# A-Nasiri-M/sap3d_tensorflow

Hardware: AMD Instinct MI355X
Metric: clips/s (16x112x112 fwd+bwd) (higher is better)
Workload: dtype f32

## Files before the change

### sap3d_tensorflow_amd/csrc/elementwise.hip

```cpp
#include "p3d_kernels.h"
#include "det_reduce.h"
#define P3D_SEED(a) ((a).seed_dev ? *(a).seed_dev : (a).seed)

namespace {

__device__ __forceinline__ float4 ld4(const float* p) { return *reinterpret_cast<const float4*>(p); }
__device__ __forceinline__ void st4(float* p, float4 v) { *reinterpret_cast<float4*>(p) = v; }
__device__ __forceinline__ float4 f4(float a) { return make_float4(a, a, a, a); }
__device__ __forceinline__ float4 fma4(float4 a, float4 b, float4 c) {
    return make_float4(fmaf(a.x, b.x, c.x), fmaf(a.y, b.y, c.y), fmaf(a.z, b.z, c.z), fmaf(a.w, b.w, c.w));
}
__device__ __forceinline__ float4 add4(float4 a, float4 b) { return make_float4(a.x + b.x, a.y + b.y, a.z + b.z, a.w + b.w); }
__device__ __forceinline__ float4 sub4(float4 a, float4 b) { return make_float4(a.x - b.x, a.y - b.y, a.z - b.z, a.w - b.w); }
__device__ __forceinline__ float4 mul4(float4 a, float4 b) { return make_float4(a.x * b.x, a.y * b.y, a.z * b.z, a.w * b.w); }
__device__ __forceinline__ float relu1(float v) { return v > 0.f ? v : (v != v ? v : 0.f); }
__device__ __forceinline__ float4 relu4(float4 a) { return make_float4(relu1(a.x), relu1(a.y), relu1(a.z), relu1(a.w)); }
__device__ __forceinline__ float4 gate4(float4 g, float4 pre) {
    return make_float4(pre.x > 0.f ? g.x : 0.f, pre.y > 0.f ? g.y : 0.f, pre.z > 0.f ? g.z : 0.f, pre.w > 0.f ? g.w : 0.f);
}

__device__ __forceinline__ float u01(unsigned long long seed, unsigned long long idx) {
    unsigned long long z = seed + 0x9E3779B97F4A7C15ull * (idx + 1);
    z = (z ^ (z >> 30)) * 0xBF58476D1CE4E5B9ull;
    z = (z ^ (z >> 27)) * 0x94D049BB133111EBull;
    z ^= z >> 31;
    return (float)(z >> 40) * (1.0f / 16777216.0f);
}
__device__ __forceinline__ float4 dropmask4(unsigned long long seed, long long e0, float rate, float scale) {
    return make_float4(u01(seed, e0) >= rate ? scale : 0.f, u01(seed, e0 + 1) >= rate ? scale : 0.f,
                       u01(seed, e0 + 2) >= rate ? scale : 0.f, u01(seed, e0 + 3) >= rate ? scale : 0.f);
}

static_assert(P3D_STAT_REPLICAS == 16, "finalize kernels fold 16 replicas with 4 shuffle steps");
__device__ __forceinline__ double fold16(double v) {
#pragma unroll
    for (int o = 8; o > 0; o >>= 1) v += __shfl_xor(v, o);
    return v;
}
template <int LPC>
__global__ __launch_bounds__(256) void bn_finalize_kernel(BnParams bn, double invM, int use_batch, int update_moving, float eps) {
    P3D_CHAIN_PRIO();
    const int r = threadIdx.x % LPC;
    const int c = blockIdx.x * (256 / LPC) + threadIdx.x / LPC;
    const bool ok = c < bn.C;
    double s1 = 0.0, s2 = 0.0;
    if (use_batch) {
        if (ok) {
            const float2* part = reinterpret_cast<const float2*>(bn.statpart) + c;
#pragma unroll 4
            for (int q = r; q < bn.nparts; q += LPC) {
                const float2 v = part[(size_t)q * bn.C];
                s1 += (double)v.x; s2 += (double)v.y;
            }
        }
#pragma unroll
        for (int o = LPC / 2; o > 0; o >>= 1) { s1 += __shfl_xor(s1, o); s2 += __shfl_xor(s2, o); }
    }
    if (!ok || r) return;
    double mean, var;
    if (use_batch) {
        mean = s1 * invM;
        var = s2 * invM - mean * mean;
        if (var < 0.0) var = 0.0;
        if (update_moving) {
            bn.moving_mean[c] -= (bn.moving_mean[c] - (float)mean) * (1.0f - 0.99f);
            bn.moving_var[c] -= (bn.moving_var[c] - (float)var) * (1.0f - 0.99f);
        }
    } else {
        mean = bn.moving_mean[c];
        var = bn.moving_var[c];
    }
    const double inv = 1.0 / sqrt(var + (double)eps);
    const float sc = (float)((double)bn.gamma[c] * inv);
    bn.scale[c] = sc;
    bn.shift[c] = (float)((double)bn.beta[c] - mean * (double)bn.gamma[c] * inv);
    bn.mean[c] = (float)mean;
    bn.invstd[c] = (float)inv;
}

__global__ __launch_bounds__(256) void bn_stats_kernel(const float* y, int ld, long long M, int C, float* statpart) {
    P3D_CHAIN_PRIO();
    __shared__ float red[256][8];
    const int c4n = C >> 2;
    const int rpi = 256 / c4n;
    const int tid = threadIdx.x;
    const int sub = tid / c4n;
    const int cg = tid - sub * c4n;
    const int c = cg << 2;
    float4 s1 = f4(0.f), s2 = f4(0.f);
    if (sub < rpi)
        for (long long row = (long long)blockIdx.x * rpi + sub; row < M; row += (long long)gridDim.x * rpi) {
            const float4 v = ld4(y + row * ld + c);
            s1 = add4(s1, v);
            s2 = fma4(v, v, s2);
        }
    float* r = red[tid];
    r[0] = s1.x; r[1] = s1.y; r[2] = s1.z; r[3] = s1.w; r[4] = s2.x; r[5] = s2.y; r[6] = s2.z; r[7] = s2.w;
    __syncthreads();
    if (tid < c4n) {
        float t[8];
#pragma unroll
        for (int q = 0; q < 8; ++q) t[q] = 0.f;
        for (int s = 0; s < rpi; ++s)
#pragma unroll
            for (int q = 0; q < 8; ++q) t[q] += red[s * c4n + tid][q];
        float* st = statpart + (size_t)blockIdx.x * 2 * C;
#pragma unroll
        for (int q = 0; q < 4; ++q) { st[2 * (c + q) + 0] = t[q]; st[2 * (c + q) + 1] = t[4 + q]; }
    }
}

template <int MODE>
__global__ __launch_bounds__(256) void bn_apply_kernel(BnApplyArgs a) {
    p3d_warm_kernarg_lines<(int)(sizeof(BnApplyArgs) / 64)>();
    P3D_CHAIN_PRIO();
    const int c4n = a.C >> 2;
    const long long total = a.M * c4n;
    for (long long i = (long long)blockIdx.x * blockDim.x + threadIdx.x; i < total; i += (long long)gridDim.x * blockDim.x) {
        const long long row = i / c4n;
        const int c = (int)(i - row * c4n) << 2;
        float4 v = fma4(ld4(a.scale1 + c), ld4(a.y1 + row * a.ld1 + c), ld4(a.shift1 + c));
        float4 z;
        if (MODE == 0) z = relu4(v);
        else if (MODE == 1) z = relu4(add4(v, ld4(a.y2 + row * a.ld2 + c)));
        else if (MODE == 2) z = relu4(add4(v, fma4(ld4(a.scale2 + c), ld4(a.y2 + row * a.ld2 + c), ld4(a.shift2 + c))));
        else if (MODE == 3) z = add4(relu4(v), relu4(fma4(ld4(a.scale2 + c), ld4(a.y2 + row * a.ld2 + c), ld4(a.shift2 + c))));
        else z = add4(ld4(a.y2 + row * a.ld2 + c), relu4(v));
        if (a.drop_scale > 0.f) z = mul4(z, dropmask4(P3D_SEED(a), row * a.C + c, a.drop_rate, a.drop_scale));
        st4(a.z + row * a.ldz + c, z);
    }
}

__device__ __forceinline__ void bn_fold64(const BnParams& bn, int c0, double invM, int use_batch, int update_moving, float eps, bool publish,
                                          float* sc_lds, float* sh_lds) {
    const int ch = c0 + (threadIdx.x >> 2), r = threadIdx.x & 3;
    double s1 = 0.0, s2 = 0.0;
    if (use_batch) {
        const float2* part = reinterpret_cast<const float2*>(bn.statpart) + ch;
#pragma unroll 8
        for (int q = r; q < bn.nparts; q += 4) {
            const float2 v = part[(size_t)q * bn.C];
            s1 += (double)v.x; s2 += (double)v.y;
        }
        s1 += __shfl_xor(s1, 1); s2 += __shfl_xor(s2, 1);
        s1 += __shfl_xor(s1, 2); s2 += __shfl_xor(s2, 2);
    }
    if (r) return;
    double mean, var;
    if (use_batch) {
        mean = s1 * invM;
        var = s2 * invM - mean * mean;
        if (var < 0.0) var = 0.0;
        if (publish && update_moving) {
            bn.moving_mean[ch] -= (bn.moving_mean[ch] - (float)mean) * (1.0f - 0.99f);
            bn.moving_var[ch] -= (bn.moving_var[ch] - (float)var) * (1.0f - 0.99f);
        }
    } else {
        mean = bn.moving_mean[ch];
        var = bn.moving_var[ch];
    }
    const double inv = 1.0 / sqrt(var + (double)eps);
    const float sc = (float)((double)bn.gamma[ch] * inv);
    const float sh = (float)((double)bn.beta[ch] - mean * (double)bn.gamma[ch] * inv);
    sc_lds[ch - c0] = sc; sh_lds[ch - c0] = sh;
    if (publish) { bn.scale[ch] = sc; bn.shift[ch] = sh; bn.mean[ch] = (float)mean; bn.invstd[ch] = (float)inv; }
}

template <int MODE>
__global__ __launch_bounds__(256) void bn_fold_apply_kernel(BnApplyArgs a, BnParams bn1, BnParams bn2, double invM, int batch1, int batch2,
                                                           int update_moving, float eps, int rows_per_block) {
    p3d_warm_kernarg_lines<(int)((sizeof(BnApplyArgs) + 2 * sizeof(BnParams)) / 64)>();
    P3D_CHAIN_PRIO();
    constexpr bool TWO = (MODE == 2 || MODE == 3);
    __shared__ __attribute__((aligned(16))) float sc1[64], sh1[64], sc2[64], sh2[64];
    const int c0 = blockIdx.y * 64;
    const bool publish = blockIdx.x == 0;
    bn_fold64(bn1, c0, invM, batch1, update_moving, eps, publish, sc1, sh1);
    if (TWO) bn_fold64(bn2, c0, invM, batch2, update_moving, eps, publish, sc2, sh2);
    __syncthreads();
    const int cl = (threadIdx.x & 15) << 2, c = c0 + cl;
    const float4 s1v = ld4(sc1 + cl), h1v = ld4(sh1 + cl);
    float4 s2v = f4(0.f), h2v = f4(0.f);
    if (TWO) { s2v = ld4(sc2 + cl); h2v = ld4(sh2 + cl); }
    const long long r0 = (long long)blockIdx.x * rows_per_block;
    const long long r1 = r0 + rows_per_block < a.M ? r0 + rows_per_block : a.M;
    for (long long row = r0 + (threadIdx.x >> 4); row < r1; row += 16) {
        const float4 v = fma4(s1v, ld4(a.y1 + row * a.ld1 + c), h1v);
        float4 z;
        if (MODE == 0) z = relu4(v);
        else if (MODE == 1) z = relu4(add4(v, ld4(a.y2 + row * a.ld2 + c)));
        else if (MODE == 2) z = relu4(add4(v, fma4(s2v, ld4(a.y2 + row * a.ld2 + c), h2v)));
        else if (MODE == 3) z = add4(relu4(v), relu4(fma4(s2v, ld4(a.y2 + row * a.ld2 + c), h2v)));
        else z = add4(ld4(a.y2 + row * a.ld2 + c), relu4(v));
        st4(a.z + row * a.ldz + c, z);
    }
}

template <int MODE>
__device__ __forceinline__ void bn_bwd_gates(const BnBwdArgs& a, long long row, int c, float4& g1, float4& g2,
                                             float4& y1, float4& y2) {
    float4 dz = ld4(a.dz + row * a.lddz + c);
    if (a.drop_scale > 0.f) dz = mul4(dz, dropmask4(P3D_SEED(a), row * a.C + c, a.drop_rate, a.drop_scale));
    y1 = ld4(a.y1 + row * a.ld1 + c);
    const float4 v1 = fma4(ld4(a.scale1 + c), y1, ld4(a.shift1 + c));
    y2 = f4(0.f);
    if (MODE == 0) { g1 = gate4(dz, v1); g2 = f4(0.f); }
    else if (MODE == 1) { y2 = ld4(a.y2 + row * a.ld2 + c); g1 = gate4(dz, add4(v1, y2)); g2 = g1; }
    else if (MODE == 2) {
        y2 = ld4(a.y2 + row * a.ld2 + c);
        const float4 v2 = fma4(ld4(a.scale2 + c), y2, ld4(a.shift2 + c));
        g1 = gate4(dz, add4(v1, v2)); g2 = g1;
    } else if (MODE == 3) {
        y2 = ld4(a.y2 + row * a.ld2 + c);
        const float4 v2 = fma4(ld4(a.scale2 + c), y2, ld4(a.shift2 + c));
        g1 = gate4(dz, v1); g2 = gate4(dz, v2);
    } else { g1 = gate4(dz, v1); g2 = dz; }
}

template <int MODE>
__global__ __launch_bounds__(256) void bn_bwd_reduce_kernel(BnBwdArgs a) {
    p3d_warm_kernarg_lines<(int)(sizeof(BnBwdArgs) / 64)>();
    P3D_CHAIN_PRIO();
    constexpr bool TWO = (MODE == 2 || MODE == 3);
    __shared__ float red[256][TWO ? 16 : 8];
    const int c4n = a.C >> 2;
    const int rpi = 256 / c4n;
    const int tid = threadIdx.x;
    const int sub = tid / c4n;
    const int cg = tid - sub * c4n;
    const int c = cg << 2;
    const bool active = sub < rpi;
    float4 s1 = f4(0.f), sx1 = f4(0.f), s2 = f4(0.f), sx2 = f4(0.f);
    if (active) {
        const float4 m1 = ld4(a.mean1 + c), i1 = ld4(a.invstd1 + c);
        float4 m2 = f4(0.f), i2 = f4(0.f);
        if (TWO) { m2 = ld4(a.mean2 + c); i2 = ld4(a.invstd2 + c); }
        const long long stride = (long long)gridDim.x * rpi;
        float4 t1 = f4(0.f), tx1 = f4(0.f), t2 = f4(0.f), tx2 = f4(0.f);
        long long row = (long long)blockIdx.x * rpi + sub;
        for (; row + stride < a.M; row += 2 * stride) {
            float4 g1, g2, y1, y2, h1, h2, z1, z2;
            bn_bwd_gates<MODE>(a, row, c, g1, g2, y1, y2);
            bn_bwd_gates<MODE>(a, row + stride, c, h1, h2, z1, z2);
            s1 = add4(s1, g1);
            sx1 = fma4(g1, mul4(sub4(y1, m1), i1), sx1);
            t1 = add4(t1, h1);
            tx1 = fma4(h1, mul4(sub4(z1, m1), i1), tx1);
            if (TWO) {
                s2 = add4(s2, g2);
                sx2 = fma4(g2, mul4(sub4(y2, m2), i2), sx2);
                t2 = add4(t2, h2);
                tx2 = fma4(h2, mul4(sub4(z2, m2), i2), tx2);
            }
        }
        if (row < a.M) {
            float4 g1, g2, y1, y2;
            bn_bwd_gates<MODE>(a, row, c, g1, g2, y1, y2);
            s1 = add4(s1, g1);
            sx1 = fma4(g1, mul4(sub4(y1, m1), i1), sx1);
            if (TWO) {
                s2 = add4(s2, g2);
                sx2 = fma4(g2, mul4(sub4(y2, m2), i2), sx2);
            }
        }
        s1 = add4(s1, t1); sx1 = add4(sx1, tx1);
        if (TWO) { s2 = add4(s2, t2); sx2 = add4(sx2, tx2); }
    }
    float* r = red[tid];
    r[0] = s1.x; r[1] = s1.y; r[2] = s1.z; r[3] = s1.w; r[4] = sx1.x; r[5] = sx1.y; r[6] = sx1.z; r[7] = sx1.w;
    if (TWO) { r[8] = s2.x; r[9] = s2.y; r[10] = s2.z; r[11] = s2.w; r[12] = sx2.x; r[13] = sx2.y; r[14] = sx2.z; r[15] = sx2.w; }
    __syncthreads();
    if (tid < c4n) {
        constexpr int NV = TWO ? 16 : 8;
        float t[NV];
#pragma unroll
        for (int q = 0; q < NV; ++q) t[q] = 0.f;
        for (int s = 0; s < rpi; ++s)
#pragma unroll
            for (int q = 0; q < NV; ++q) t[q] += red[s * c4n + tid][q];
        float* p1 = a.part1 + ((size_t)blockIdx.x * a.C + c) * 2;
#pragma unroll
        for (int q = 0; q < 4; ++q) { p1[2 * q] = t[q]; p1[2 * q + 1] = t[4 + q]; }
        if (TWO) {
            float* p2 = a.part2 + ((size_t)blockIdx.x * a.C + c) * 2;
#pragma unroll
            for (int q = 0; q < 4; ++q) { p2[2 * q] = t[8 + q]; p2[2 * q + 1] = t[12 + q]; }
        }
    }
}

template <int LPC>
__global__ __launch_bounds__(256) void bn_bwd_finalize_kernel(BnBwdArgs a, int two) {
    p3d_warm_kernarg_lines<(int)(sizeof(BnBwdArgs) / 64)>();
    P3D_CHAIN_PRIO();
    const int r = threadIdx.x % LPC;
    const int c = blockIdx.x * (256 / LPC) + threadIdx.x / LPC;
    const bool ok = c < a.C;
    const double invM = 1.0 / (double)a.M;
    double s1 = 0.0, s2 = 0.0, t1 = 0.0, t2 = 0.0;
    if (ok) {
        const float2* p1 = reinterpret_cast<const float2*>(a.part1) + c;
        const float2* p2 = reinterpret_cast<const float2*>(a.part2) + c;
#pragma unroll 4
        for (int q = r; q < a.nparts; q += LPC) {
            const float2 v = p1[(size_t)q * a.C];
            s1 += (double)v.x; s2 += (double)v.y;
            if (two) { const float2 w = p2[(size_t)q * a.C]; t1 += (double)w.x; t2 += (double)w.y; }
        }
    }
#pragma unroll
    for (int o = LPC / 2; o > 0; o >>= 1) {
        s1 += __shfl_xor(s1, o); s2 += __shfl_xor(s2, o);
        if (two) { t1 += __shfl_xor(t1, o); t2 += __shfl_xor(t2, o); }
    }
    if (!ok || r) return;
    a.dbeta1[c] = (float)s1; a.dgamma1[c] = (float)s2;
    a.coef1[2 * c] = (float)(s1 * invM); a.coef1[2 * c + 1] = (float)(s2 * invM);
    if (two) {
        a.dbeta2[c] = (float)t1; a.dgamma2[c] = (float)t2;
        a.coef2[2 * c] = (float)(t1 * invM); a.coef2[2 * c + 1] = (float)(t2 * invM);
    }
}

__global__ __launch_bounds__(256) void bn_grad_finalize_kernel(BnGradFold f) {
    P3D_CHAIN_PRIO();
    const int r = threadIdx.x & 15;
    const int c = blockIdx.x * 16 + (threadIdx.x >> 4);
    const bool ok = c < f.C;
    double sg = 0.0, sgx = 0.0;
    if (ok) {
        const float2* part = reinterpret_cast<const float2*>(f.part) + c;
#pragma unroll 4
        for (int q = r; q < f.nparts; q += 16) {
            const float2 v = part[(size_t)q * f.C];
            sg += (double)v.x; sgx += (double)v.y;
        }
    }
    sg = fold16(sg); sgx = fold16(sgx);
    if (!ok || r) return;
    const float inv = f.invstd[c];
    const float c1 = (float)(sg * f.inv_m), c2 = (float)(sgx * f.inv_m);
    const float k1 = f.gamma[c] * inv;
    const float k2 = -k1 * inv * c2;
    const float k3 = -k1 * c1 - k2 * f.mean[c];
    f.coef[c] = k1; f.coef[f.C + c] = k2; f.coef[2 * f.C + c] = k3;
    f.dgamma[c] = (float)sgx; f.dbeta[c] = (float)sg;
}

__device__ __forceinline__ void ldcoef(const float* coef, int c, float4& c1, float4& c2) {
    const float4 lo = ld4(coef + 2 * c), hi = ld4(coef + 2 * c + 4);
    c1 = make_float4(lo.x, lo.z, hi.x, hi.z);
    c2 = make_float4(lo.y, lo.w, hi.y, hi.w);
}

template <int MODE>
__global__ __launch_bounds__(256) void bn_bwd_apply_kernel(BnBwdArgs a) {
    p3d_warm_kernarg_lines<(int)(sizeof(BnBwdArgs) / 64)>();
    P3D_CHAIN_PRIO();
    constexpr bool TWO = (MODE == 2 || MODE == 3);
    const int c4n = a.C >> 2;
    const long long total = a.M * c4n;
    const long long gtid = (long long)blockIdx.x * blockDim.x + threadIdx.x;
    for (long long i = gtid; i < total; i += (long long)gridDim.x * blockDim.x) {
        const long long row = i / c4n;
        const int c = (int)(i - row * c4n) << 2;
        float4 g1, g2, y1, y2;
        bn_bwd_gates<MODE>(a, row, c, g1, g2, y1, y2);
        {
            const float4 k = mul4(ld4(a.gamma1 + c), ld4(a.invstd1 + c));
            float4 d;
            if (a.batch1) {
                const float4 xh = mul4(sub4(y1, ld4(a.mean1 + c)), ld4(a.invstd1 + c));
                float4 c1, c2;
                ldcoef(a.coef1, c, c1, c2);
                d = mul4(k, sub4(sub4(g1, c1), mul4(xh, c2)));
            } else d = mul4(k, g1);
            float* dst = a.dy1 + row * a.lddy1 + c;
            if (a.acc1) d = add4(d, ld4(dst));
            st4(dst, d);
        }
        if (MODE != 0) {
            float4 d;
            if (TWO) {
                const float4 k = mul4(ld4(a.gamma2 + c), ld4(a.invstd2 + c));
                if (a.batch2) {
                    const float4 xh = mul4(sub4(y2, ld4(a.mean2 + c)), ld4(a.invstd2 + c));
                    float4 c1, c2;
                    ldcoef(a.coef2, c, c1, c2);
                    d = mul4(k, sub4(sub4(g2, c1), mul4(xh, c2)));
                } else d = mul4(k, g2);
            } else d = g2;
            float* dst = a.dy2 + row * a.lddy2 + c;
            if (a.acc2) d = add4(d, ld4(dst));
            st4(dst, d);
        }
    }
}

__global__ __launch_bounds__(256) void maxpool_fwd_kernel(PoolArgs a) {
    p3d_warm_kernarg_lines<(int)(sizeof(PoolArgs) / 64)>();
    P3D_CHAIN_PRIO();
    const int c4n = a.C >> 2;
    const long long total = (long long)a.N * a.Do * a.Ho * a.Wo * c4n;
    for (long long i = (long long)blockIdx.x * blockDim.x + threadIdx.x; i < total; i += (long long)gridDim.x * blockDim.x) {
        long long pos = i / c4n;
        const int c = (int)(i - pos * c4n) << 2;
        const long long opos = pos;
        const int ow = (int)(pos % a.Wo); pos /= a.Wo;
        const int oh = (int)(pos % a.Ho); pos /= a.Ho;
        const int od = (int)(pos % a.Do); const int n = (int)(pos / a.Do);
        float4 best = f4(-INFINITY);
        unsigned bx = 0, by = 0, bz = 0, bw = 0;
        bool none = true;
        for (int kd = 0; kd < a.kd; ++kd) {
            const int id = od * a.sd - a.pd + kd;
            if ((unsigned)id >= (unsigned)a.Di) continue;
            for (int kh = 0; kh < a.kh; ++kh) {
                const int ih = oh * a.sh - a.ph + kh;
                if ((unsigned)ih >= (unsigned)a.Hi) continue;
                for (int kw = 0; kw < a.kw; ++kw) {
                    const int iw = ow * a.sw - a.pw + kw;
                    if ((unsigned)iw >= (unsigned)a.Wi) continue;
                    const float4 v = ld4(a.x + ((((long long)n * a.Di + id) * a.Hi + ih) * a.Wi + iw) * a.ldx + c);
                    const unsigned t = (unsigned)((kd * a.kh + kh) * a.kw + kw);
                    if (none || v.x > best.x || (v.x != v.x && best.x == best.x)) { best.x = v.x; bx = t; }
                    if (none || v.y > best.y || (v.y != v.y && best.y == best.y)) { best.y = v.y; by = t; }
                    if (none || v.z > best.z || (v.z != v.z && best.z == best.z)) { best.z = v.z; bz = t; }
                    if (none || v.w > best.w || (v.w != v.w && best.w == best.w)) { best.w = v.w; bw = t; }
                    none = false;
                }
            }
        }
        st4(a.y + opos * a.ldy + c, best);
        if (a.idx) a.idx[opos * c4n + (c >> 2)] = bx | (by << 8) | (bz << 16) | (bw << 24);
    }
}

template <int KIND>
__device__ __forceinline__ float loss_term(float z, float p, float t, int through_sigmoid, float& g) {
    if (KIND == 1) {
        g = (through_sigmoid ? p : 1.f / (1.f + expf(-z))) - t;
        return fmaxf(z, 0.f) - z * t + log1pf(expf(-fabsf(z)));
    }
    const float d = p - t;
    const float ad = fabsf(d);
    const bool quad = KIND == 0 && ad < 1.f;
    g = quad ? d : (d > 0.f ? 1.f : (d < 0.f ? -1.f : (d != d ? d : 0.f)));
    if (through_sigmoid) g *= p * (1.f - p);
    return KIND == 2 ? ad : (quad ? 0.5f * d * d : ad - 0.5f);
}

template <int KIND>
__device__ __forceinline__ void loss_body(const float* logits, const float* pred, const float* target, long long n,
                                          double* loss_out, float* dl, int through_sigmoid, int vec4, double* part,
                                          unsigned* counter) {
    __shared__ double wsum[4];
    __shared__ int last_flag;
    double acc = 0.0;
    const bool need_z = KIND == 1, need_p = KIND != 1 || through_sigmoid;
    const long long gtid = (long long)blockIdx.x * blockDim.x + threadIdx.x, gsz = (long long)gridDim.x * blockDim.x;
// ... 269 lines not shown
        for (long long e = a + threadIdx.x; e < a4; e += 256) one(e);
        for (long long e = b4 + threadIdx.x; e < b; e += 256) one(e);
        acc = p3d_block_sum<true>(acc, wsum);
        if (threadIdx.x == 0) p3d_store_wt(part, (size_t)k, acc);
    }
    if (nfold <= 0) return;
    if (!p3d_last_block_wt(counter, gridDim.x, &last_flag)) return;
    double s = 0.0;
    for (int k = threadIdx.x; k < nfold; k += 256) s += part[k];
    const double sumsq = p3d_block_sum<true>(s, wsum);
    if (threadIdx.x == 0) {
        const double norm = sqrt(sumsq), cn = (double)clip;
        float scale;
        if (!(norm - norm == 0.0)) scale = __builtin_nanf("");
        else if (cn - cn != 0.0) scale = 1.f;
        else scale = (float)(cn / fmax(norm, cn));
        res[0] = sumsq; res[1] = norm;
        *reinterpret_cast<float*>(res + 2) = scale;
    }
}

__global__ __launch_bounds__(256) void add_inplace_kernel(float* dst, int lddst, const float* src, int ldsrc, long long M, int C, int copy) {
    const int c4n = C >> 2;
    const long long total = M * c4n;
    for (long long i = (long long)blockIdx.x * blockDim.x + threadIdx.x; i < total; i += (long long)gridDim.x * blockDim.x) {
        const long long row = i / c4n;
        const int c = (int)(i - row * c4n) << 2;
        float4 v = ld4(src + row * ldsrc + c);
        if (!copy) v = add4(v, ld4(dst + row * lddst + c));
        st4(dst + row * lddst + c, v);
    }
}

__global__ __launch_bounds__(256) void fill_uniform_kernel(float* p, long long n, float lo, float hi, unsigned long long seed) {
    for (long long i = (long long)blockIdx.x * blockDim.x + threadIdx.x; i < n; i += (long long)gridDim.x * blockDim.x)
        p[i] = lo + (hi - lo) * u01(seed, (unsigned long long)i);
}

__global__ __launch_bounds__(256) void fill_trunc_normal_kernel(float* p, long long n, float stddev, unsigned long long seed) {
    for (long long i = (long long)blockIdx.x * blockDim.x + threadIdx.x; i < n; i += (long long)gridDim.x * blockDim.x) {
        float z = 0.f;
        for (int k = 0; k < 32; ++k) {
            const unsigned long long e = 2ull * (unsigned long long)(i + (long long)k * n);
            const float u1 = fmaxf(u01(seed, e), 1e-12f), u2 = u01(seed, e + 1);
            z = sqrtf(-2.f * logf(u1)) * cosf(6.2831853071795865f * u2);
            if (fabsf(z) <= 2.f) break;
            z = 0.f;
        }
        p[i] = stddev * z;
    }
}

__global__ __launch_bounds__(256) void colsum_kernel(const float* dy, int ld, long long M, int C, float* out, float* part,
                                                     unsigned* counters) {
    __shared__ int last_flag;
    const int c = blockIdx.y * blockDim.x + threadIdx.x;
    float acc = 0.f;
    if (c < C) {
        long long row = blockIdx.x;
        const long long st = gridDim.x;
        for (; row + 7 * st < M; row += 8 * st) {
            float v[8];
#pragma unroll
            for (int u = 0; u < 8; ++u) v[u] = dy[(row + u * st) * ld + c];
#pragma unroll
            for (int u = 0; u < 8; ++u) acc += v[u];
        }
        for (; row < M; row += st) acc += dy[row * ld + c];
        p3d_store_wt(part, (size_t)blockIdx.x * C + c, acc);
    }
    if (!p3d_last_block_wt(counters + blockIdx.y, gridDim.x, &last_flag)) return;
    if (c >= C) return;
    float t = 0.f;
    unsigned b = 0;
    for (; b + 7 < gridDim.x; b += 8) {
        float v[8];
#pragma unroll
        for (int u = 0; u < 8; ++u) v[u] = part[(size_t)(b + u) * C + c];
#pragma unroll
        for (int u = 0; u < 8; ++u) t += v[u];
    }
    for (; b < gridDim.x; ++b) t += part[(size_t)b * C + c];
    out[c] += t;
}

__global__ __launch_bounds__(256) void colsum4_kernel(const float* __restrict__ dy, int ld, long long M, int C, float* out,
                                                      float* part, unsigned* counters) {
    __shared__ float4 red[256];
    __shared__ int last_flag;
    const int L = C >> 2, R = 256 / L;
    const int lane = threadIdx.x % L, rs = threadIdx.x / L;
    const bool live = rs < R;
    float4 acc = make_float4(0.f, 0.f, 0.f, 0.f);
    if (live) {
        const long long stride = (long long)gridDim.x * R;
        long long row = (long long)blockIdx.x * R + rs;
        const float* base = dy + lane * 4;
        for (; row + 7 * stride < M; row += 8 * stride) {
            float4 v[8];
#pragma unroll
            for (int u = 0; u < 8; ++u) v[u] = *reinterpret_cast<const float4*>(base + (row + u * stride) * ld);
#pragma unroll
            for (int u = 0; u < 8; ++u) { acc.x += v[u].x; acc.y += v[u].y; acc.z += v[u].z; acc.w += v[u].w; }
        }
        for (; row < M; row += stride) {
            const float4 v = *reinterpret_cast<const float4*>(base + row * ld);
            acc.x += v.x; acc.y += v.y; acc.z += v.z; acc.w += v.w;
        }
    }
    red[threadIdx.x] = acc;
    __syncthreads();
    if (threadIdx.x < L) {
        float4 t = red[threadIdx.x];
        for (int r = 1; r < R; ++r) { const float4 v = red[r * L + threadIdx.x]; t.x += v.x; t.y += v.y; t.z += v.z; t.w += v.w; }
        p3d_store_wt4(part, (size_t)blockIdx.x * C + threadIdx.x * 4, t);
    }
    if (!p3d_last_block_wt(counters, gridDim.x, &last_flag)) return;
    acc = make_float4(0.f, 0.f, 0.f, 0.f);
    if (live) {
        const float* src = part + lane * 4;
        unsigned b = rs;
        for (; b + 7u * R < gridDim.x; b += 8u * R) {
            float4 v[8];
#pragma unroll
            for (int u = 0; u < 8; ++u) v[u] = *reinterpret_cast<const float4*>(src + (size_t)(b + u * R) * C);
#pragma unroll
            for (int u = 0; u < 8; ++u) { acc.x += v[u].x; acc.y += v[u].y; acc.z += v[u].z; acc.w += v[u].w; }
        }
        for (; b < gridDim.x; b += R) {
            const float4 v = *reinterpret_cast<const float4*>(src + (size_t)b * C);
            acc.x += v.x; acc.y += v.y; acc.z += v.z; acc.w += v.w;
        }
    }
    __syncthreads();
    red[threadIdx.x] = acc;
    __syncthreads();
    if (threadIdx.x < L) {
        float4 t = red[threadIdx.x];
        for (int r = 1; r < R; ++r) { const float4 v = red[r * L + threadIdx.x]; t.x += v.x; t.y += v.y; t.z += v.z; t.w += v.w; }
        float4* o = reinterpret_cast<float4*>(out + threadIdx.x * 4);
        float4 cur = *o;
        cur.x += t.x; cur.y += t.y; cur.z += t.z; cur.w += t.w;
        *o = cur;
    }
}

inline unsigned grid_for(long long total, int per_block = 256, int cap = 4096) {
    long long b = (total + per_block - 1) / per_block;
    if (b < 1) b = 1;
    if (b > cap) b = cap;
    return (unsigned)b;
}

}

hipError_t p3d_bn_finalize(const BnParams& bn, long M, int use_batch, int update_moving, float eps, hipStream_t s) {
    if (use_batch && (!bn.statpart || bn.nparts < 1)) return hipErrorInvalidValue;
    if (use_batch && bn.nparts > 64)
        hipLaunchKernelGGL(bn_finalize_kernel<64>, dim3((bn.C + 3) / 4), dim3(256), 0, s, bn, 1.0 / (double)M, use_batch, update_moving, eps);
    else
        hipLaunchKernelGGL(bn_finalize_kernel<16>, dim3((bn.C + 15) / 16), dim3(256), 0, s, bn, 1.0 / (double)M, use_batch, update_moving, eps);
    return hipGetLastError();
}

int p3d_bn_stats_parts(long M, int C) {
    if ((C & 3) || C > 1024 || C < 4) return 0;
    const int rpi = 256 / (C >> 2);
    long long blocks = (M + (long long)rpi * 8 - 1) / ((long long)rpi * 8);
    if (blocks < 1) blocks = 1;
    if (blocks > 512) blocks = 512;
    return (int)blocks;
}

hipError_t p3d_bn_stats(const float* y, int ld, long M, int C, float* statpart, hipStream_t s) {
    if ((C & 3) || C > 1024 || (ld & 3)) return hipErrorInvalidValue;
    const long long blocks = p3d_bn_stats_parts(M, C);
    hipLaunchKernelGGL(bn_stats_kernel, dim3((unsigned)blocks), dim3(256), 0, s, y, ld, (long long)M, C, statpart);
    return hipGetLastError();
}

hipError_t p3d_bn_apply(const BnApplyArgs& a, hipStream_t s) {
    if ((a.C & 3) || (a.ld1 & 3) || (a.ldz & 3)) return hipErrorInvalidValue;
    const unsigned g = grid_for(a.M * (a.C >> 2));
    switch (a.mode) {
        case 0: hipLaunchKernelGGL(bn_apply_kernel<0>, dim3(g), dim3(256), 0, s, a); break;
        case 1: hipLaunchKernelGGL(bn_apply_kernel<1>, dim3(g), dim3(256), 0, s, a); break;
        case 2: hipLaunchKernelGGL(bn_apply_kernel<2>, dim3(g), dim3(256), 0, s, a); break;
        case 3: hipLaunchKernelGGL(bn_apply_kernel<3>, dim3(g), dim3(256), 0, s, a); break;
        case 4: hipLaunchKernelGGL(bn_apply_kernel<4>, dim3(g), dim3(256), 0, s, a); break;
        default: return hipErrorInvalidValue;
    }
    return hipGetLastError();
}

bool p3d_bn_fold_apply_ok(long M, int C, int nparts1, int nparts2, float drop_scale) {
    static const bool off = p3d_tune_env("P3D_BN_FOLD_APPLY") && atoi(p3d_tune_env("P3D_BN_FOLD_APPLY")) == 0;
    return !off && (C % 64) == 0 && nparts1 <= 128 && nparts2 <= 128 && M >= 1024 && !(drop_scale > 0.f);
}
hipError_t p3d_bn_fold_apply(const BnApplyArgs& a, const BnParams& bn1, const BnParams& bn2, int batch1, int batch2, int update_moving,
                             float eps, hipStream_t s) {
    const bool two = a.mode == 2 || a.mode == 3;
    if ((a.ld1 & 3) || (a.ldz & 3) || !p3d_bn_fold_apply_ok(a.M, a.C, batch1 ? bn1.nparts : 0, two && batch2 ? bn2.nparts : 0, a.drop_scale))
        return hipErrorInvalidValue;
    if ((batch1 && (!bn1.statpart || bn1.nparts < 1)) || (two && batch2 && (!bn2.statpart || bn2.nparts < 1))) return hipErrorInvalidValue;
    const int groups = a.C / 64;
    int chunks = 256 / groups;
    if (chunks < 1) chunks = 1;
    long rows = (a.M + chunks - 1) / chunks;
    rows = (rows + 15) / 16 * 16;
    chunks = (int)((a.M + rows - 1) / rows);
    const dim3 g((unsigned)chunks, (unsigned)groups);
    const double invM = 1.0 / (double)a.M;
#define P3D_FA(M_) case M_: hipLaunchKernelGGL(bn_fold_apply_kernel<M_>, g, dim3(256), 0, s, a, bn1, bn2, invM, batch1, batch2, update_moving, eps, (int)rows); break;
    switch (a.mode) { P3D_FA(0) P3D_FA(1) P3D_FA(2) P3D_FA(3) P3D_FA(4) default: return hipErrorInvalidValue; }
#undef P3D_FA
    return hipGetLastError();
}

int p3d_bn_bwd_parts(long M, int C) {
    if ((C & 3) || C > 1024 || C < 4) return 0;
    const int rpi = 256 / (C >> 2);
    long long blocks = (M + (long long)rpi * 8 - 1) / ((long long)rpi * 8);
    if (blocks < 1) blocks = 1;
    if (blocks > 512) blocks = 512;
    return (int)blocks;
}

hipError_t p3d_bn_bwd_reduce(const BnBwdArgs& a, hipStream_t s) {
    if ((a.C & 3) || a.C > 1024 || !a.part1 || a.nparts != p3d_bn_bwd_parts(a.M, a.C)) return hipErrorInvalidValue;
    const unsigned g = (unsigned)a.nparts;
    switch (a.mode) {
        case 0: hipLaunchKernelGGL(bn_bwd_reduce_kernel<0>, dim3(g), dim3(256), 0, s, a); break;
        case 1: hipLaunchKernelGGL(bn_bwd_reduce_kernel<1>, dim3(g), dim3(256), 0, s, a); break;
        case 2: hipLaunchKernelGGL(bn_bwd_reduce_kernel<2>, dim3(g), dim3(256), 0, s, a); break;
        case 3: hipLaunchKernelGGL(bn_bwd_reduce_kernel<3>, dim3(g), dim3(256), 0, s, a); break;
        case 4: hipLaunchKernelGGL(bn_bwd_reduce_kernel<4>, dim3(g), dim3(256), 0, s, a); break;
        default: return hipErrorInvalidValue;
    }
    return hipGetLastError();
}

hipError_t p3d_bn_bwd_finalize(const BnBwdArgs& a, hipStream_t s) {
    const int two = (a.mode == 2 || a.mode == 3) ? 1 : 0;
    if (a.nparts >= 64) hipLaunchKernelGGL(bn_bwd_finalize_kernel<64>, dim3((a.C + 3) / 4), dim3(256), 0, s, a, two);
    else hipLaunchKernelGGL(bn_bwd_finalize_kernel<16>, dim3((a.C + 15) / 16), dim3(256), 0, s, a, two);
    return hipGetLastError();
}

hipError_t p3d_bn_grad_finalize(const BnGradFold& f, hipStream_t s) {
    if (!f.part || f.nparts <= 0) return hipErrorInvalidValue;
    hipLaunchKernelGGL(bn_grad_finalize_kernel, dim3((f.C + 15) / 16), dim3(256), 0, s, f);
    return hipGetLastError();
}

hipError_t p3d_bn_bwd_apply(const BnBwdArgs& a, hipStream_t s) {
    if (a.C & 3) return hipErrorInvalidValue;
    unsigned g = grid_for(a.M * (a.C >> 2));
    switch (a.mode) {
        case 0: hipLaunchKernelGGL(bn_bwd_apply_kernel<0>, dim3(g), dim3(256), 0, s, a); break;
        case 1: hipLaunchKernelGGL(bn_bwd_apply_kernel<1>, dim3(g), dim3(256), 0, s, a); break;
        case 2: hipLaunchKernelGGL(bn_bwd_apply_kernel<2>, dim3(g), dim3(256), 0, s, a); break;
        case 3: hipLaunchKernelGGL(bn_bwd_apply_kernel<3>, dim3(g), dim3(256), 0, s, a); break;
        case 4: hipLaunchKernelGGL(bn_bwd_apply_kernel<4>, dim3(g), dim3(256), 0, s, a); break;
        default: return hipErrorInvalidValue;
    }
    return hipGetLastError();
}

hipError_t p3d_maxpool_fwd(const PoolArgs& a, hipStream_t s) {
    if (a.C & 3) return hipErrorInvalidValue;
    const long long total = (long long)a.N * a.Do * a.Ho * a.Wo * (a.C >> 2);
    hipLaunchKernelGGL(maxpool_fwd_kernel, dim3(grid_for(total)), dim3(256), 0, s, a);
    return hipGetLastError();
}

__device__ __forceinline__ bool pool_hit(float v, float y) { return v == y || (v != v && y != y); }
__global__ __launch_bounds__(256) void maxpool_bwd_disjoint_kernel(PoolArgs a, int accumulate) {
    p3d_warm_kernarg_lines<(int)(sizeof(PoolArgs) / 64)>();
    P3D_CHAIN_PRIO();
    const int c4n = a.C >> 2;
    const long long total = (long long)a.N * a.Do * a.Ho * a.Wo * c4n;
    for (long long i = (long long)blockIdx.x * blockDim.x + threadIdx.x; i < total; i += (long long)gridDim.x * blockDim.x) {
        long long pos = i / c4n;
        const int c = (int)(i - pos * c4n) << 2;
        const long long opos = pos;
        const int ow = (int)(pos % a.Wo); pos /= a.Wo;
        const int oh = (int)(pos % a.Ho); pos /= a.Ho;
        const int od = (int)(pos % a.Do); const int n = (int)(pos / a.Do);
        const float4 g = ld4(a.dy + opos * a.lddy + c);
        const float4 y = ld4(a.y + opos * a.ldy + c);
        float4 left = g;
        bool done[4] = {false, false, false, false};
        for (int kd = 0; kd < a.kd; ++kd)
            for (int kh = 0; kh < a.kh; ++kh)
                for (int kw = 0; kw < a.kw; ++kw) {
                    const long long ipos = (((long long)n * a.Di + od * a.sd + kd) * a.Hi + oh * a.sh + kh) * a.Wi + ow * a.sw + kw;
                    const float4 v = ld4(a.x + ipos * a.ldx + c);
                    float4 d = f4(0.f);
                    if (!done[0] && pool_hit(v.x, y.x)) { d.x = left.x; done[0] = true; }
                    if (!done[1] && pool_hit(v.y, y.y)) { d.y = left.y; done[1] = true; }
                    if (!done[2] && pool_hit(v.z, y.z)) { d.z = left.z; done[2] = true; }
                    if (!done[3] && pool_hit(v.w, y.w)) { d.w = left.w; done[3] = true; }
                    float* dst = a.dx + ipos * a.lddx + c;
                    if (accumulate) d = add4(d, ld4(dst));
                    st4(dst, d);
                }
    }
}

__global__ __launch_bounds__(256) void maxpool_bwd_gather_kernel(PoolArgs a, int accumulate) {
    p3d_warm_kernarg_lines<(int)(sizeof(PoolArgs) / 64)>();
    P3D_CHAIN_PRIO();
    const int c4n = a.C >> 2;
    const long long total = (long long)a.N * a.Di * a.Hi * a.Wi * c4n;
    for (long long i = (long long)blockIdx.x * blockDim.x + threadIdx.x; i < total; i += (long long)gridDim.x * blockDim.x) {
        long long pos = i / c4n;
        const int c = (int)(i - pos * c4n) << 2;
        const long long ipos = pos;
        const int iw = (int)(pos % a.Wi); pos /= a.Wi;
        const int ih = (int)(pos % a.Hi); pos /= a.Hi;
        const int id = (int)(pos % a.Di); const int n = (int)(pos / a.Di);
        const int pdv = id + a.pd, phv = ih + a.ph, pwv = iw + a.pw;
        float4 acc = f4(0.f);
        if (a.kd <= 2 * a.sd && a.kh <= 2 * a.sh && a.kw <= 2 * a.sw) {
            int od2[2], oh2[2], ow2[2];
            bool vd[2], vh[2], vw[2];
#pragma unroll
            for (int q = 0; q < 2; ++q) {
                od2[q] = pdv / a.sd - q; vd[q] = od2[q] >= 0 && od2[q] < a.Do && pdv - od2[q] * a.sd < a.kd;
                oh2[q] = phv / a.sh - q; vh[q] = oh2[q] >= 0 && oh2[q] < a.Ho && phv - oh2[q] * a.sh < a.kh;
                ow2[q] = pwv / a.sw - q; vw[q] = ow2[q] >= 0 && ow2[q] < a.Wo && pwv - ow2[q] * a.sw < a.kw;
            }
            unsigned wd[8]; float4 g8[8]; unsigned t8[8]; bool ok[8];
#pragma unroll
            for (int q = 0; q < 8; ++q) {
                const int qd = q >> 2, qh = (q >> 1) & 1, qw = q & 1;
                ok[q] = vd[qd] && vh[qh] && vw[qw];
                t8[q] = (unsigned)(((pdv - od2[qd] * a.sd) * a.kh + (phv - oh2[qh] * a.sh)) * a.kw + (pwv - ow2[qw] * a.sw));
                const long long opos = ok[q] ? (((long long)n * a.Do + od2[qd]) * a.Ho + oh2[qh]) * a.Wo + ow2[qw] : 0;
                wd[q] = ok[q] ? a.idx[opos * c4n + (c >> 2)] : 0xffffffffu;
                g8[q] = ok[q] ? ld4(a.dy + opos * a.lddy + c) : f4(0.f);
            }
#pragma unroll
            for (int q = 0; q < 8; ++q) {
                if (!ok[q]) continue;
                const unsigned w = wd[q], t = t8[q];
                if ((w & 255u) == t) acc.x += g8[q].x;
                if (((w >> 8) & 255u) == t) acc.y += g8[q].y;
                if (((w >> 16) & 255u) == t) acc.z += g8[q].z;
                if ((w >> 24) == t) acc.w += g8[q].w;
            }
        } else
        for (int od = pdv / a.sd; od >= 0 && pdv - od * a.sd < a.kd; --od) {
            if (od >= a.Do) continue;
            for (int oh = phv / a.sh; oh >= 0 && phv - oh * a.sh < a.kh; --oh) {
                if (oh >= a.Ho) continue;
                for (int ow = pwv / a.sw; ow >= 0 && pwv - ow * a.sw < a.kw; --ow) {
                    if (ow >= a.Wo) continue;
                    const unsigned t = (unsigned)(((pdv - od * a.sd) * a.kh + (phv - oh * a.sh)) * a.kw + (pwv - ow * a.sw));
                    const long long opos = (((long long)n * a.Do + od) * a.Ho + oh) * a.Wo + ow;
                    const unsigned w = a.idx[opos * c4n + (c >> 2)];
                    const float4 g = ld4(a.dy + opos * a.lddy + c);
                    if ((w & 255u) == t) acc.x += g.x;
                    if (((w >> 8) & 255u) == t) acc.y += g.y;
                    if (((w >> 16) & 255u) == t) acc.z += g.z;
                    if ((w >> 24) == t) acc.w += g.w;
                }
            }
        }
        float* dst = a.dx + ipos * a.lddx + c;
        if (accumulate) acc = add4(acc, ld4(dst));
        st4(dst, acc);
    }
}

bool p3d_maxpool_disjoint(const PoolArgs& a) {
    return a.kd == a.sd && a.kh == a.sh && a.kw == a.sw && a.pd == 0 && a.ph == 0 && a.pw == 0 &&
           a.Do * a.sd == a.Di && a.Ho * a.sh == a.Hi && a.Wo * a.sw == a.Wi;
}

hipError_t p3d_maxpool_bwd_disjoint(const PoolArgs& a, int accumulate, hipStream_t s) {
    if ((a.C & 3) || !p3d_maxpool_disjoint(a)) return hipErrorInvalidValue;
    const long long total = (long long)a.N * a.Do * a.Ho * a.Wo * (a.C >> 2);
    hipLaunchKernelGGL(maxpool_bwd_disjoint_kernel, dim3(grid_for(total)), dim3(256), 0, s, a, accumulate);
    return hipGetLastError();
}


static uintptr_t low4(const void* q) { return reinterpret_cast<uintptr_t>(q) & 15; }

LaunchDesc p3d_loss_desc(const LossArgs& a) {
    const double n = (double)a.n;
    const bool ts = a.through_sigmoid != 0;
    if (a.kind == 1) return {"sigmoid_ce_kernel", n * (ts ? 8.0 : 11.0), n * (ts ? 16.0 : 12.0)};
    if (a.kind == 2) return {"l1_loss_kernel", n * (ts ? 6.0 : 3.0), n * 12.0};
    return {"smooth_l1_kernel", 0, 12.0 * n};
}

// ... 239 lines not shown
```

Before: 538.0.

## Batch BN partial-stat loads and prefetch activations ahead of stat fold

Adds specialized paths across the BN kernels that issue all partial-sum loads up front in fixed-size unrolled batches instead of a strided loop, so the finalize kernels avoid serialized memory latency. The fold-apply kernel prefetches its first activation rows before the stat fold and sync, overlapping those loads with the reduction. The backward reduce gains a short-chain path that loads up to eight rows per thread into registers before accumulating. This costs more registers and clamped redundant loads, and the new paths can be disabled by environment variables in tuning builds.

```diff
diff --git a/sap3d_tensorflow_amd/csrc/elementwise.hip b/sap3d_tensorflow_amd/csrc/elementwise.hip
--- a/sap3d_tensorflow_amd/csrc/elementwise.hip
+++ b/sap3d_tensorflow_amd/csrc/elementwise.hip
@@ -37,20 +37,51 @@
     for (int o = 8; o > 0; o >>= 1) v += __shfl_xor(v, o);
     return v;
 }
-template <int LPC>
+template <int NB, int LPC, bool TWO>
+__device__ __forceinline__ void bn_lane_batch(const float2* p1, const float2* p2, int r, int nparts, int C, double& s1, double& s2,
+                                              double& t1, double& t2) {
+    float2 v[NB], w[NB];
+#pragma unroll
+    for (int k = 0; k < NB; ++k) {
+        const int q = r + k * LPC;
+        const size_t at = (size_t)(q < nparts ? q : nparts - 1) * C;
+        v[k] = p1[at];
+        if (TWO) w[k] = p2[at];
+    }
+#pragma unroll
+    for (int k = 0; k < NB; ++k)
+        if (r + k * LPC < nparts) {
+            s1 += (double)v[k].x; s2 += (double)v[k].y;
+            if (TWO) { t1 += (double)w[k].x; t2 += (double)w[k].y; }
+        }
+}
+template <int NB0, int LPC, bool TWO>
+__device__ __forceinline__ void bn_lane_tiers(const float2* p1, const float2* p2, int r, int nparts, int C, double& s1, double& s2,
+                                              double& t1, double& t2) {
+    if (nparts <= NB0 * LPC) bn_lane_batch<NB0, LPC, TWO>(p1, p2, r, nparts, C, s1, s2, t1, t2);
+    else if (nparts <= 2 * NB0 * LPC) bn_lane_batch<2 * NB0, LPC, TWO>(p1, p2, r, nparts, C, s1, s2, t1, t2);
+    else bn_lane_batch<4 * NB0, LPC, TWO>(p1, p2, r, nparts, C, s1, s2, t1, t2);
+}
+template <int LPC, bool BATCH>
 __global__ __launch_bounds__(256) void bn_finalize_kernel(BnParams bn, double invM, int use_batch, int update_moving, float eps) {
     P3D_CHAIN_PRIO();
     const int r = threadIdx.x % LPC;
     const int c = blockIdx.x * (256 / LPC) + threadIdx.x / LPC;
     const bool ok = c < bn.C;
+    constexpr int NB0 = LPC == 64 ? 2 : 1;
     double s1 = 0.0, s2 = 0.0;
     if (use_batch) {
         if (ok) {
             const float2* part = reinterpret_cast<const float2*>(bn.statpart) + c;
+            if (BATCH && bn.nparts <= 4 * NB0 * LPC) {
+                double t1 = 0.0, t2 = 0.0;
+                bn_lane_tiers<NB0, LPC, false>(part, part, r, bn.nparts, bn.C, s1, s2, t1, t2);
+            } else {
 #pragma unroll 4
-            for (int q = r; q < bn.nparts; q += LPC) {
-                const float2 v = part[(size_t)q * bn.C];
-                s1 += (double)v.x; s2 += (double)v.y;
+                for (int q = r; q < bn.nparts; q += LPC) {
+                    const float2 v = part[(size_t)q * bn.C];
+                    s1 += (double)v.x; s2 += (double)v.y;
+                }
             }
         }
 #pragma unroll
@@ -132,15 +163,20 @@
 }
 
 __device__ __forceinline__ void bn_fold64(const BnParams& bn, int c0, double invM, int use_batch, int update_moving, float eps, bool publish,
-                                          float* sc_lds, float* sh_lds) {
+                                          float* sc_lds, float* sh_lds, bool batch) {
     const int ch = c0 + (threadIdx.x >> 2), r = threadIdx.x & 3;
     double s1 = 0.0, s2 = 0.0;
     if (use_batch) {
         const float2* part = reinterpret_cast<const float2*>(bn.statpart) + ch;
+        if (batch && bn.nparts <= 128) {
+            double t1 = 0.0, t2 = 0.0;
+            bn_lane_tiers<8, 4, false>(part, part, r, bn.nparts, bn.C, s1, s2, t1, t2);
+        } else {
 #pragma unroll 8
-        for (int q = r; q < bn.nparts; q += 4) {
-            const float2 v = part[(size_t)q * bn.C];
-            s1 += (double)v.x; s2 += (double)v.y;
+            for (int q = r; q < bn.nparts; q += 4) {
+                const float2 v = part[(size_t)q * bn.C];
+                s1 += (double)v.x; s2 += (double)v.y;
+            }
         }
         s1 += __shfl_xor(s1, 1); s2 += __shfl_xor(s2, 1);
         s1 += __shfl_xor(s1, 2); s2 += __shfl_xor(s2, 2);
@@ -167,32 +203,60 @@
 }
 
 template <int MODE>
+__device__ __forceinline__ float4 bn_apply_z(float4 y1, float4 y2, float4 s1v, float4 h1v, float4 s2v, float4 h2v) {
+    const float4 v = fma4(s1v, y1, h1v);
+    if (MODE == 0) return relu4(v);
+    else if (MODE == 1) return relu4(add4(v, y2));
+    else if (MODE == 2) return relu4(add4(v, fma4(s2v, y2, h2v)));
+    else if (MODE == 3) return add4(relu4(v), relu4(fma4(s2v, y2, h2v)));
+    else return add4(y2, relu4(v));
+}
+
+template <int MODE, bool EARLY>
 __global__ __launch_bounds__(256) void bn_fold_apply_kernel(BnApplyArgs a, BnParams bn1, BnParams bn2, double invM, int batch1, int batch2,
                                                            int update_moving, float eps, int rows_per_block) {
     p3d_warm_kernarg_lines<(int)((sizeof(BnApplyArgs) + 2 * sizeof(BnParams)) / 64)>();
     P3D_CHAIN_PRIO();
     constexpr bool TWO = (MODE == 2 || MODE == 3);
+    constexpr int PRE = 4;
     __shared__ __attribute__((aligned(16))) float sc1[64], sh1[64], sc2[64], sh2[64];
     const int c0 = blockIdx.y * 64;
     const bool publish = blockIdx.x == 0;
-    bn_fold64(bn1, c0, invM, batch1, update_moving, eps, publish, sc1, sh1);
-    if (TWO) bn_fold64(bn2, c0, invM, batch2, update_moving, eps, publish, sc2, sh2);
+    const int cl = (threadIdx.x & 15) << 2, c = c0 + cl;
+    const long long r0 = (long long)blockIdx.x * rows_per_block;
+    const long long r1 = r0 + rows_per_block < a.M ? r0 + rows_per_block : a.M;
+    long long row = r0 + (threadIdx.x >> 4);
+    float4 py1[PRE], py2[PRE];
+    auto load_trips = [&]() {
+#pragma unroll
+        for (int k = 0; k < PRE; ++k) {
+            const long long rk = row + 16 * k < r1 ? row + 16 * k : r1 - 1;
+            py1[k] = ld4(a.y1 + rk * a.ld1 + c);
+            py2[k] = MODE != 0 ? ld4(a.y2 + rk * a.ld2 + c) : f4(0.f);
+        }
+    };
+    if (EARLY) load_trips();
+    bn_fold64(bn1, c0, invM, batch1, update_moving, eps, publish, sc1, sh1, EARLY);
+    if (TWO) bn_fold64(bn2, c0, invM, batch2, update_moving, eps, publish, sc2, sh2, EARLY);
     __syncthreads();
-    const int cl = (threadIdx.x & 15) << 2, c = c0 + cl;
     const float4 s1v = ld4(sc1 + cl), h1v = ld4(sh1 + cl);
     float4 s2v = f4(0.f), h2v = f4(0.f);
     if (TWO) { s2v = ld4(sc2 + cl); h2v = ld4(sh2 + cl); }
-    const long long r0 = (long long)blockIdx.x * rows_per_block;
-    const long long r1 = r0 + rows_per_block < a.M ? r0 + rows_per_block : a.M;
-    for (long long row = r0 + (threadIdx.x >> 4); row < r1; row += 16) {
-        const float4 v = fma4(s1v, ld4(a.y1 + row * a.ld1 + c), h1v);
-        float4 z;
-        if (MODE == 0) z = relu4(v);
-        else if (MODE == 1) z = relu4(add4(v, ld4(a.y2 + row * a.ld2 + c)));
-        else if (MODE == 2) z = relu4(add4(v, fma4(s2v, ld4(a.y2 + row * a.ld2 + c), h2v)));
-        else if (MODE == 3) z = add4(relu4(v), relu4(fma4(s2v, ld4(a.y2 + row * a.ld2 + c), h2v)));
-        else z = add4(ld4(a.y2 + row * a.ld2 + c), relu4(v));
-        st4(a.z + row * a.ldz + c, z);
+    if (EARLY) {
+        for (;;) {
+#pragma unroll
+            for (int k = 0; k < PRE; ++k)
+                if (row + 16 * k < r1) st4(a.z + (row + 16 * k) * a.ldz + c, bn_apply_z<MODE>(py1[k], py2[k], s1v, h1v, s2v, h2v));
+            row += 16 * PRE;
+            if (row >= r1) break;
+            load_trips();
+        }
+        return;
+    }
+    for (; row < r1; row += 16) {
+        const float4 y1 = ld4(a.y1 + row * a.ld1 + c);
+        const float4 y2 = MODE != 0 ? ld4(a.y2 + row * a.ld2 + c) : f4(0.f);
+        st4(a.z + row * a.ldz + c, bn_apply_z<MODE>(y1, y2, s1v, h1v, s2v, h2v));
     }
 }
 
@@ -216,8 +280,19 @@
         g1 = gate4(dz, v1); g2 = gate4(dz, v2);
     } else { g1 = gate4(dz, v1); g2 = dz; }
 }
-
 template <int MODE>
+__device__ __forceinline__ void bn_bwd_gates_reg(float4 dz, float4 y1, float4 y2, const float4 (&sv)[4], float4& g1, float4& g2) {
+    const float4 v1 = fma4(sv[0], y1, sv[1]);
+    if (MODE == 0) { g1 = gate4(dz, v1); g2 = f4(0.f); }
+    else if (MODE == 1) { g1 = gate4(dz, add4(v1, y2)); g2 = g1; }
+    else if (MODE == 2) { g1 = gate4(dz, add4(v1, fma4(sv[2], y2, sv[3]))); g2 = g1; }
+    else if (MODE == 3) { g1 = gate4(dz, v1); g2 = gate4(dz, fma4(sv[2], y2, sv[3])); }
+    else { g1 = gate4(dz, v1); g2 = dz; }
+}
+
+#define P3D_BN_REDUCE_SHORT_GRID 256
+#define P3D_BN_REDUCE_SHORT 8
+template <int MODE, bool SHORT>
 __global__ __launch_bounds__(256) void bn_bwd_reduce_kernel(BnBwdArgs a) {
     p3d_warm_kernarg_lines<(int)(sizeof(BnBwdArgs) / 64)>();
     P3D_CHAIN_PRIO();
@@ -238,6 +313,34 @@
         const long long stride = (long long)gridDim.x * rpi;
         float4 t1 = f4(0.f), tx1 = f4(0.f), t2 = f4(0.f), tx2 = f4(0.f);
         long long row = (long long)blockIdx.x * rpi + sub;
+        if (SHORT && !(a.drop_scale > 0.f) && a.M <= P3D_BN_REDUCE_SHORT * stride && gridDim.x <= P3D_BN_REDUCE_SHORT_GRID) {
+            float4 dz[P3D_BN_REDUCE_SHORT], y1[P3D_BN_REDUCE_SHORT], y2[P3D_BN_REDUCE_SHORT], sv[4];
+#pragma unroll
+            for (int k = 0; k < P3D_BN_REDUCE_SHORT; ++k) {
+                const long long rk = row + k * stride < a.M ? row + k * stride : a.M - 1;
+                dz[k] = ld4(a.dz + rk * a.lddz + c);
+                y1[k] = ld4(a.y1 + rk * a.ld1 + c);
+                y2[k] = MODE != 0 ? ld4(a.y2 + rk * a.ld2 + c) : f4(0.f);
+            }
+            sv[0] = ld4(a.scale1 + c); sv[1] = ld4(a.shift1 + c);
+            sv[2] = TWO ? ld4(a.scale2 + c) : f4(0.f); sv[3] = TWO ? ld4(a.shift2 + c) : f4(0.f);
+#pragma unroll
+            for (int k = 0; k < P3D_BN_REDUCE_SHORT; ++k)
+                if (row + k * stride < a.M) {
+                    float4 g1, g2;
+                    bn_bwd_gates_reg<MODE>(dz[k], y1[k], y2[k], sv, g1, g2);
+                    if (k & 1) {
+                        t1 = add4(t1, g1);
+                        tx1 = fma4(g1, mul4(sub4(y1[k], m1), i1), tx1);
+                        if (TWO) { t2 = add4(t2, g2); tx2 = fma4(g2, mul4(sub4(y2[k], m2), i2), tx2); }
+                    } else {
+                        s1 = add4(s1, g1);
+                        sx1 = fma4(g1, mul4(sub4(y1[k], m1), i1), sx1);
+                        if (TWO) { s2 = add4(s2, g2); sx2 = fma4(g2, mul4(sub4(y2[k], m2), i2), sx2); }
+                    }
+                }
+            row = a.M;
+        }
         for (; row + stride < a.M; row += 2 * stride) {
             float4 g1, g2, y1, y2, h1, h2, z1, z2;
             bn_bwd_gates<MODE>(a, row, c, g1, g2, y1, y2);
@@ -289,7 +392,7 @@
     }
 }
 
-template <int LPC>
+template <int LPC, bool BATCH>
 __global__ __launch_bounds__(256) void bn_bwd_finalize_kernel(BnBwdArgs a, int two) {
     p3d_warm_kernarg_lines<(int)(sizeof(BnBwdArgs) / 64)>();
     P3D_CHAIN_PRIO();
@@ -297,15 +400,21 @@
     const int c = blockIdx.x * (256 / LPC) + threadIdx.x / LPC;
     const bool ok = c < a.C;
     const double invM = 1.0 / (double)a.M;
+    constexpr int NB0 = LPC == 64 ? 2 : 1;
     double s1 = 0.0, s2 = 0.0, t1 = 0.0, t2 = 0.0;
     if (ok) {
         const float2* p1 = reinterpret_cast<const float2*>(a.part1) + c;
         const float2* p2 = reinterpret_cast<const float2*>(a.part2) + c;
+        if (BATCH && a.nparts <= 4 * NB0 * LPC) {
+            if (two) bn_lane_tiers<NB0, LPC, true>(p1, p2, r, a.nparts, a.C, s1, s2, t1, t2);
+            else bn_lane_tiers<NB0, LPC, false>(p1, p1, r, a.nparts, a.C, s1, s2, t1, t2);
+        } else {
 #pragma unroll 4
-        for (int q = r; q < a.nparts; q += LPC) {
-            const float2 v = p1[(size_t)q * a.C];
-            s1 += (double)v.x; s2 += (double)v.y;
-            if (two) { const float2 w = p2[(size_t)q * a.C]; t1 += (double)w.x; t2 += (double)w.y; }
+            for (int q = r; q < a.nparts; q += LPC) {
+                const float2 v = p1[(size_t)q * a.C];
+                s1 += (double)v.x; s2 += (double)v.y;
+                if (two) { const float2 w = p2[(size_t)q * a.C]; t1 += (double)w.x; t2 += (double)w.y; }
+            }
         }
     }
 #pragma unroll
@@ -881,14 +990,22 @@
     return (unsigned)b;
 }
 
+#if defined(P3D_TUNING)
+inline bool bn_path_off(const char* name) { const char* e = p3d_tune_env(name); return e && atoi(e) == 0; }
+#else
+inline bool bn_path_off(const char*) { return false; }
+#endif
+#define P3D_BN_PICK(NAME, TAKES, ...) do { \
+        if ((TAKES) && !bn_path_off(NAME)) { constexpr bool PATH_ = true; __VA_ARGS__; } else { constexpr bool PATH_ = false; __VA_ARGS__; } } while (0)
+
 }
 
 hipError_t p3d_bn_finalize(const BnParams& bn, long M, int use_batch, int update_moving, float eps, hipStream_t s) {
     if (use_batch && (!bn.statpart || bn.nparts < 1)) return hipErrorInvalidValue;
     if (use_batch && bn.nparts > 64)
-        hipLaunchKernelGGL(bn_finalize_kernel<64>, dim3((bn.C + 3) / 4), dim3(256), 0, s, bn, 1.0 / (double)M, use_batch, update_moving, eps);
+        P3D_BN_PICK("P3D_BN_FINALIZE_BATCH", bn.nparts <= 512, hipLaunchKernelGGL((bn_finalize_kernel<64, PATH_>), dim3((bn.C + 3) / 4), dim3(256), 0, s, bn, 1.0 / (double)M, use_batch, update_moving, eps));
     else
-        hipLaunchKernelGGL(bn_finalize_kernel<16>, dim3((bn.C + 15) / 16), dim3(256), 0, s, bn, 1.0 / (double)M, use_batch, update_moving, eps);
+        P3D_BN_PICK("P3D_BN_FINALIZE_BATCH", use_batch && bn.nparts <= 64, hipLaunchKernelGGL((bn_finalize_kernel<16, PATH_>), dim3((bn.C + 15) / 16), dim3(256), 0, s, bn, 1.0 / (double)M, use_batch, update_moving, eps));
     return hipGetLastError();
 }
 
@@ -940,7 +1057,7 @@
     chunks = (int)((a.M + rows - 1) / rows);
     const dim3 g((unsigned)chunks, (unsigned)groups);
     const double invM = 1.0 / (double)a.M;
-#define P3D_FA(M_) case M_: hipLaunchKernelGGL(bn_fold_apply_kernel<M_>, g, dim3(256), 0, s, a, bn1, bn2, invM, batch1, batch2, update_moving, eps, (int)rows); break;
+#define P3D_FA(M_) case M_: P3D_BN_PICK("P3D_BN_FOLD_EARLY", rows > 64, hipLaunchKernelGGL((bn_fold_apply_kernel<M_, PATH_>), g, dim3(256), 0, s, a, bn1, bn2, invM, batch1, batch2, update_moving, eps, (int)rows)); break;
     switch (a.mode) { P3D_FA(0) P3D_FA(1) P3D_FA(2) P3D_FA(3) P3D_FA(4) default: return hipErrorInvalidValue; }
 #undef P3D_FA
     return hipGetLastError();
@@ -958,12 +1075,13 @@
 hipError_t p3d_bn_bwd_reduce(const BnBwdArgs& a, hipStream_t s) {
     if ((a.C & 3) || a.C > 1024 || !a.part1 || a.nparts != p3d_bn_bwd_parts(a.M, a.C)) return hipErrorInvalidValue;
     const unsigned g = (unsigned)a.nparts;
+    const bool short_chain = a.M <= (long long)P3D_BN_REDUCE_SHORT * g * (256 / (a.C >> 2)) && g <= P3D_BN_REDUCE_SHORT_GRID && !(a.drop_scale > 0.f);
     switch (a.mode) {
-        case 0: hipLaunchKernelGGL(bn_bwd_reduce_kernel<0>, dim3(g), dim3(256), 0, s, a); break;
-        case 1: hipLaunchKernelGGL(bn_bwd_reduce_kernel<1>, dim3(g), dim3(256), 0, s, a); break;
-        case 2: hipLaunchKernelGGL(bn_bwd_reduce_kernel<2>, dim3(g), dim3(256), 0, s, a); break;
-        case 3: hipLaunchKernelGGL(bn_bwd_reduce_kernel<3>, dim3(g), dim3(256), 0, s, a); break;
-        case 4: hipLaunchKernelGGL(bn_bwd_reduce_kernel<4>, dim3(g), dim3(256), 0, s, a); break;
+        case 0: P3D_BN_PICK("P3D_BN_REDUCE_SHORT", short_chain, hipLaunchKernelGGL((bn_bwd_reduce_kernel<0, PATH_>), dim3(g), dim3(256), 0, s, a)); break;
+        case 1: P3D_BN_PICK("P3D_BN_REDUCE_SHORT", short_chain, hipLaunchKernelGGL((bn_bwd_reduce_kernel<1, PATH_>), dim3(g), dim3(256), 0, s, a)); break;
+        case 2: P3D_BN_PICK("P3D_BN_REDUCE_SHORT", short_chain, hipLaunchKernelGGL((bn_bwd_reduce_kernel<2, PATH_>), dim3(g), dim3(256), 0, s, a)); break;
+        case 3: P3D_BN_PICK("P3D_BN_REDUCE_SHORT", short_chain, hipLaunchKernelGGL((bn_bwd_reduce_kernel<3, PATH_>), dim3(g), dim3(256), 0, s, a)); break;
+        case 4: P3D_BN_PICK("P3D_BN_REDUCE_SHORT", short_chain, hipLaunchKernelGGL((bn_bwd_reduce_kernel<4, PATH_>), dim3(g), dim3(256), 0, s, a)); break;
         default: return hipErrorInvalidValue;
     }
     return hipGetLastError();
@@ -971,8 +1089,8 @@
 
 hipError_t p3d_bn_bwd_finalize(const BnBwdArgs& a, hipStream_t s) {
     const int two = (a.mode == 2 || a.mode == 3) ? 1 : 0;
-    if (a.nparts >= 64) hipLaunchKernelGGL(bn_bwd_finalize_kernel<64>, dim3((a.C + 3) / 4), dim3(256), 0, s, a, two);
-    else hipLaunchKernelGGL(bn_bwd_finalize_kernel<16>, dim3((a.C + 15) / 16), dim3(256), 0, s, a, two);
+    if (a.nparts >= 64) P3D_BN_PICK("P3D_BN_FINALIZE_BATCH", a.nparts <= (two ? 256 : 512), hipLaunchKernelGGL((bn_bwd_finalize_kernel<64, PATH_>), dim3((a.C + 3) / 4), dim3(256), 0, s, a, two));
+    else P3D_BN_PICK("P3D_BN_FINALIZE_BATCH", true, hipLaunchKernelGGL((bn_bwd_finalize_kernel<16, PATH_>), dim3((a.C + 15) / 16), dim3(256), 0, s, a, two));
     return hipGetLastError();
 }
 
```

Result: no change. 538.4, median of 2 (+0.1%).
